# input-output-hk/plutus-halo2-verifier-gen

Hardware: AMD Instinct MI355X
Metric: halo2_proofs_verified_per_sec (higher is better)
Workload: dtype u32

## Files before the change

plutus_halo2_verifier_gen_amd/csrc/h2v_capi.hip:

```cpp
#include "../../include/h2v.h"

#include <hip/hip_runtime.h>
#include <stdio.h>
#include <stdlib.h>
#include <string.h>

#include <mutex>
#include <string>
#include <vector>

#include "h2v_kernels.hip"
#include "h2v_plancc.hpp"

static thread_local std::string g_err;
static int fail(int code, const std::string &msg) {
    g_err = msg;
    if (code == H2V_E_DEVICE && msg.find("hip: ") == std::string::npos) {
        const hipError_t e = hipPeekAtLastError();
        if (e != hipSuccess) g_err += std::string(" [hip: ") + hipGetErrorString(e) + "]";
    }
    return code;
}
#define HIPCHK(expr)                                                                                     \
    do {                                                                                                 \
// ... 53 lines not shown
        return fail(H2V_E_ARG, std::string("verifying-key description: ") + e.what());
    } catch (const std::exception &e) {
        return fail(H2V_E_ARG, std::string("plan compiler: ") + e.what());
    }
}
extern "C" void h2v_blob_free(uint8_t *blob) { free(blob); }

struct h2v_plan {
    int device = 0;
    bool dead = false;
    H2vDevPlan d{};
    void *blob = nullptr;
    void *fold_terms = nullptr;
    void *vk_tab = nullptr;
    void *fix_tab = nullptr;
    uint32_t n_var = 0, n_fix = 0;
    uint32_t n_squeezes = 0, stream_len = 0;
    uint64_t gen = 0;
    std::vector<uint32_t> trace_slots;
};

struct h2v_workspace {
    int device = 0;
    bool dead = false;
    uint32_t in_flight_hint = 1;
    bool hint_given = false;
    uint64_t cap = 0;
    uint32_t stride = 0;
    uint32_t sz_terms = 0, sz_slots = 0, sz_regs = 0 , sz_trace = 0;
    bool sz_ivc = false, sz_fix = false;
    uint32_t *regs = nullptr, *scalars = nullptr, *pts = nullptr, *er = nullptr, *status = nullptr, *trace = nullptr, *msm_tab = nullptr;
    uint32_t *accl = nullptr, *accr = nullptr, *fold_pts = nullptr, *fold_scal = nullptr, *el2 = nullptr, *er2 = nullptr;
    uint32_t *pt_tab = nullptr;
    uint32_t *er_fix = nullptr;
    uint32_t *msm_parts = nullptr;
// ... 264 lines not shown
        if (p->vk_tab) (void)hipFree(p->vk_tab);
        if (p->fold_terms) (void)hipFree(p->fold_terms);
        (void)hipFree(p->blob); delete p;
        return fail(H2V_E_DEVICE, "hipMalloc(vk tables) failed");
    }
    if (n_bases) {
        hipLaunchKernelGGL(k_vk_tables, dim3((n_bases + 63) / 64), dim3(64), 0, nullptr, d.vk_bases, n_bases, (uint32_t *)p->vk_tab);
        if (hipDeviceSynchronize() != hipSuccess) {
            (void)hipFree(p->vk_tab);
            if (p->fold_terms) (void)hipFree(p->fold_terms);
            (void)hipFree(p->blob); delete p;
            return fail(H2V_E_DEVICE, "VK window-table kernel failed");
        }
    }
    d.vk_tab = (const uint32_t *)p->vk_tab;
    if (!ivc && n_bases) {
        uint32_t nv = 0;
        while (nv < n_terms && rd32(patched.data() + w[H2V_HW_OFF_TERMS] + 8 * nv) != H2V_TERM_VK_BASE) nv++;
        bool tail_ok = nv < n_terms;
        for (uint32_t k = nv; k < n_terms; k++) tail_ok = tail_ok && rd32(patched.data() + w[H2V_HW_OFF_TERMS] + 8 * k) == H2V_TERM_VK_BASE;
        if (tail_ok) {
            uint32_t fc = (size_t)n_bases * 22 * 2048 * 112 <= ((size_t)2 << 30) ? 12u : 8u;
            if (opt_fix_c) fc = opt_fix_c;
            const uint32_t fW = fc == 4 ? 65u : fc == 8 ? 33u : 22u, fE = 1u << (fc - 1);
            const size_t fix_bytes = (size_t)n_bases * fW * fE * 28 * 4;
            void *wbase = nullptr;
            bool okf = hipMalloc(&p->fix_tab, fix_bytes + 16) == hipSuccess && hipMemset(p->fix_tab, 0, fix_bytes + 16) == hipSuccess &&
                       hipMalloc(&wbase, (size_t)n_bases * fW * 96 + 16) == hipSuccess;
            if (okf) {
                hipLaunchKernelGGL(k_vk_fixed_window_bases, dim3((n_bases * fW + 63) / 64), dim3(64), 0, nullptr, d.vk_bases, n_bases, fc, fW, (uint32_t *)wbase);
                const uint64_t entries = (uint64_t)n_bases * fW * fE;
                hipLaunchKernelGGL(k_vk_fixed_tables, dim3((uint32_t)((entries + 63) / 64)), dim3(64), 0, nullptr, (const uint32_t *)wbase, n_bases * fW, fc, (uint32_t *)p->fix_tab);
                okf = hipDeviceSynchronize() == hipSuccess;
            }
            if (wbase) (void)hipFree(wbase);
            d.fix_c = fc; d.fix_W = fW;
            if (!okf) {
                if (p->fix_tab) (void)hipFree(p->fix_tab);
                (void)hipFree(p->vk_tab);
                (void)hipFree(p->blob); delete p;
                return fail(H2V_E_DEVICE, "fixed-base table setup failed");
            }
            p->n_var = nv;
            p->n_fix = n_terms - nv;
        }
    }
    d.fix_tab = (const uint32_t *)p->fix_tab; d.n_var = p->n_var; d.n_fix = p->n_fix;
    p->n_squeezes = n_sq;
    p->stream_len = w[H2V_HW_STREAM_LEN];
    for (uint32_t k = 0; k < n_trace; k++) p->trace_slots.push_back(rd32(trp + 8 * k));
    { static std::mutex mu; static uint64_t loads = 0; std::lock_guard<std::mutex> lock(mu); p->gen = ++loads; }
    reg_add(g_plan_live, p);
    *out = p;
    return H2V_OK;
}
static void plan_release(h2v_plan *p) {
    (void)hipSetDevice(p->device);
    if (p->blob) (void)hipFree(p->blob);
    if (p->fold_terms) (void)hipFree(p->fold_terms);
    if (p->vk_tab) (void)hipFree(p->vk_tab);
    if (p->fix_tab) (void)hipFree(p->fix_tab);
    p->blob = p->fold_terms = p->vk_tab = p->fix_tab = nullptr;
}
extern "C" void h2v_plan_free(h2v_plan *p) {
    if (!p) return;
    reg_del(g_plan_live, p);
    if (!p->dead) plan_release(p);
    delete p;
}
extern "C" int h2v_plan_info(const h2v_plan *p, uint32_t *proof_len, uint32_t *n_pi, uint32_t *n_ci, uint32_t *n_terms) {
    if (!p) return fail(H2V_E_ARG, "null plan");
    if (proof_len) *proof_len = p->d.proof_len;
    if (n_pi) *n_pi = p->d.n_pi;
    if (n_ci) *n_ci = p->d.n_ci;
    if (n_terms) *n_terms = p->d.n_terms;
    return H2V_OK;
}
// ... 614 lines not shown
    return launch_msm_range(d, ma, n, scalars, pts, nullptr, st, in_flight_hint, seg);
}
struct IvcBufs { uint32_t *accl, *accr, *fold_pts, *fold_scal, *el2, *er2; };
static void launch_ivc_fold(const H2vDevPlan &d, uint32_t n, const uint32_t *pts, const uint32_t *er,
                            const IvcBufs &b, uint32_t *tabws, hipStream_t st) {
    hipLaunchKernelGGL(k_ivc_challenge, dim3((n + 63) / 64), dim3(64), 0, st, d, n, pts, er, b.accl, b.accr, b.fold_pts, b.fold_scal);
    const H2vMsmArgs fold = {d.fold_terms, 0, 4, 4, 0, 4, {2, 4, 4}, {b.el2, b.er2, nullptr}, nullptr, nullptr, nullptr, 0, 0};
    launch_msm_range(d, fold, n, b.fold_scal, b.fold_pts, tabws, st);
}
static uint32_t launch_pairing_impl(int impl, const H2vDevPlan &d, uint32_t n, const uint32_t *pts, const uint8_t *valid, const uint8_t *valid_sub, const uint32_t *er,
                                const uint32_t *el_jac, uint32_t *status, uint8_t *accept, uint32_t *dbg, hipStream_t st, const uint32_t *skip = nullptr,
                                bool prefer_narrow = false, double wide_up_to = -1.0, bool prefer_six = false, bool prefer_twelve = false) {
    if (wide_up_to < 0) wide_up_to = msm_n_simd();
    const int forced = g_opts.v[H2V_OPT_PAIRING_ENGINE];
    if (impl == 1 && forced) impl = forced == 1 ? 0 : forced == 16 ? 2 : forced == 64 ? 3 : forced == 6 ? 5 : forced == 12 ? 6 : 4;
    if (impl == 5 || (impl == 1 && !skip && prefer_six)) {
        hipLaunchKernelGGL(k_pairing_six, dim3((n + SIX_GROUPS - 1) / SIX_GROUPS), dim3(64), SIX_LDS_BYTES, st, d, n, pts, valid, valid_sub, er, el_jac, status, accept, dbg);
        return 6u;
    }
    const bool wide = !skip && impl != 2 && impl != 4 && impl != 6 && (impl == 3 || (double)n <= wide_up_to);
    const bool narrow = !skip && !wide && impl != 4 && (impl == 2 || prefer_narrow);
    if (impl == 6 || (narrow && impl != 2 && prefer_twelve)) {
        hipLaunchKernelGGL(k_pairing_coop_twelve, dim3((n + COOP_GROUPS_TWELVE - 1) / COOP_GROUPS_TWELVE), dim3(64), COOP_LDS_BYTES(COOP_GROUPS_TWELVE), st, d, n, pts, valid, valid_sub, er, el_jac, status, accept, dbg);
        return 12u;
    }
    if (impl == 0) { hipLaunchKernelGGL(k_pairing_check, dim3((n + 63) / 64), dim3(64), 0, st, d, n, pts, valid, valid_sub, er, el_jac, status, accept, dbg); return 1; }
    else if (wide) hipLaunchKernelGGL(k_pairing_coop_wide, dim3(n), dim3(64), COOP_LDS_BYTES(1), st, d, n, pts, valid, valid_sub, er, el_jac, status, accept, dbg);
    else if (narrow) hipLaunchKernelGGL(k_pairing_coop_narrow, dim3((n + 3) / 4), dim3(64), COOP_LDS_BYTES(COOP_GROUPS_NARROW), st, d, n, pts, valid, valid_sub, er, el_jac, status, accept, dbg);
    else hipLaunchKernelGGL(k_pairing_coop, dim3((n + 1) / 2), dim3(64), COOP_LDS_BYTES(COOP_GROUPS_PER_WAVE), st, d, n, pts, valid, valid_sub, er, el_jac, status, accept, dbg, skip);
    return wide ? 64u : narrow ? 16u : 32u;
}
// ... 1600 lines not shown
}
extern "C" int h2v_probe_pairing_ex(const h2v_plan *p, uint32_t n, const uint8_t *p1c, const uint8_t *p2c, uint8_t *out, int impl, uint8_t *dbg);
extern "C" int h2v_probe_pairing(const h2v_plan *p, uint32_t n, const uint8_t *p1c, const uint8_t *p2c, uint8_t *out) {
    return h2v_probe_pairing_ex(p, n, p1c, p2c, out, -1, nullptr);
}
extern "C" int h2v_probe_pairing_ex(const h2v_plan *p, uint32_t n, const uint8_t *p1c, const uint8_t *p2c, uint8_t *out, int impl, uint8_t *dbg) {
    if (!p || !p1c || !p2c || !out || n == 0) return fail(H2V_E_ARG, "bad argument");
    ALIVE(p);
    ProbeOpts probe_opts;
    DevBuf ddbg;
    HIPCHK(hipSetDevice(p->device));
    MiniPlan mp;
    DevBuf din, doff, dsc, dpts, dvalid, der, dst, dacc, dtab;
    mp.d.lines28_sg2 = p->d.lines28_sg2;
    mp.d.lines28_g2 = p->d.lines28_g2;
    if (mp.build(2, 1, p->d.lines_sg2, p->d.lines_g2) || upload_offsets(doff, n, 96) || din.alloc((size_t)n * 96) || dsc.alloc((size_t)n * 32) ||
        dpts.alloc((size_t)n * 192) || dvalid.alloc((size_t)n * 2) || der.alloc((size_t)n * 144) || dst.alloc((size_t)n * 4) || dacc.alloc(n))
        return fail(H2V_E_DEVICE, "probe setup failed");
    uint32_t term[2] = {H2V_TERM_PROOF_POINT, 1};
    HIPCHK(hipMemcpy(mp.terms.p, term, 8, hipMemcpyHostToDevice));
    std::vector<uint8_t> in((size_t)n * 96), one((size_t)n * 32, 0);
    for (uint32_t i = 0; i < n; i++) { memcpy(&in[(size_t)i * 96], p1c + (size_t)i * 48, 48); memcpy(&in[(size_t)i * 96 + 48], p2c + (size_t)i * 48, 48); one[(size_t)i * 32] = 1; }
    HIPCHK(hipMemcpy(din.p, in.data(), in.size(), hipMemcpyHostToDevice));
    HIPCHK(hipMemcpy(dsc.p, one.data(), one.size(), hipMemcpyHostToDevice));
    HIPCHK(hipMemset(dst.p, 0, (size_t)n * 4));
    if (dtab.alloc((size_t)n * 2 * 448 * 4)) return fail(H2V_E_DEVICE, "hipMalloc failed");
    hipLaunchKernelGGL(k_g1_decompress, dim3((n * 2 + 63) / 64), dim3(128), 0, nullptr, mp.d, n, din.as<uint8_t>(), doff.as<uint64_t>(), (const uint8_t *)nullptr, (const uint8_t *)nullptr, dpts.as<uint32_t>(), dvalid.as<uint8_t>(), dtab.as<uint32_t>(), 0u, (uint8_t *)nullptr);
    launch_msm(mp.d, n, dsc.as<uint32_t>(), dpts.as<uint32_t>(), dtab.as<uint32_t>(), der.as<uint32_t>(), nullptr, nullptr, nullptr);
    if (ddbg.alloc(dbg ? (size_t)n * 24 * 48 : 8)) return fail(H2V_E_DEVICE, "hipMalloc failed");
    launch_pairing_impl(impl, mp.d, n, dpts.as<uint32_t>(), dvalid.as<uint8_t>(), nullptr, der.as<uint32_t>(), nullptr, dst.as<uint32_t>(), dacc.as<uint8_t>(), dbg ? ddbg.as<uint32_t>() : nullptr, nullptr);
// ... 7 lines not shown
```

plutus_halo2_verifier_gen_amd/csrc/h2v_curve28.hpp:

```cpp
#pragma once
#include "h2v_curve.hpp"
#include "h2v_fp28.hpp"

struct G1J28 { F28 x, y, z; };

H2V_DI void g1j28_from_affine(G1J28 &r, const G1A &a) {
    f28_from_fp(r.x, a.x);
    f28_from_fp(r.y, a.y);
    f28_set_one(r.z);
}
H2V_DI void g1j28_to_g1j(G1J &r, const G1J28 &p, const bool inf) {
    if (inf) { g1j_set_inf(r); return; }
    F28 z = p.z;
    f28_carry(z);
    f28_to_fp(r.x, p.x);
    f28_to_fp(r.y, p.y);
    f28_to_fp(r.z, z);
}
#define F28_MUL_(r, a, b) do { if (INL) f28_mul_inl(r, a, b); else f28_mul(r, a, b); } while (0)
#define F28_SQR_(r, a) do { if (INL) f28_sqr_inl(r, a); else f28_sqr(r, a); } while (0)
template <bool INL>
H2V_DI void g1j28_dbl_t(G1J28 &r, const G1J28 &p) {
    F28 X = p.x, Y = p.y, Z = p.z, A, B, D, t;
    F28_NEG(t, Y, 21, 1);
// ... 3 lines not shown
    F28_MUL_(D, X, B);
    f28_mul_small<3>(A, A);
    F28_SQR_(X, A);
    f28_mul_small<8>(t, D);
    F28_SUB(X, X, t, 17, 8); f28_carry(X);
    f28_mul_small<4>(D, D);
    F28_SUB(t, X, D, 9, 4); f28_carry(t);
    f28_mul_small<2>(B, B);
    if (INL) f28_dot2_sqr_inl<2>(Y, B, A, t);
    else f28_dot2_sqr<2>(Y, B, A, t);
    r.x = X; r.y = Y; r.z = Z;
}
#undef F28_MUL_
#undef F28_SQR_
H2V_DI void g1j28_dbl(G1J28 &r, const G1J28 &p) { g1j28_dbl_t<false>(r, p); }
H2V_DI int g1j28_add(G1J28 &r, const G1J28 &p, const G1J28 &q, const bool neg_q) {
    F28 X1 = p.x, Y1 = p.y, Z1 = p.z, a, b, c, t;
    f28_sqr(a, q.z);
    f28_mul(X1, X1, a);
    f28_mul(t, q.z, a); f28_mul(Y1, Y1, t);
    f28_sqr(a, Z1);
    f28_mul(b, q.x, a);
    f28_mul(t, Z1, a);
    {
        F28 qy = q.y, nq;
        F28_NEG(nq, qy, 20, 1);
        if (neg_q) qy = nq;
        f28_mul(c, qy, t);
    }
    F28_SUB(b, b, X1, 3, 1); f28_carry(b);
    F28_SUB(c, Y1, c, 3, 1); f28_carry(c);
    if (f28_is_zero_v5(b)) {
        if (f28_is_zero_v5(c)) { g1j28_dbl(r, p); return 1; }
        return 2;
    }
    f28_mul(Z1, Z1, q.z); f28_mul(Z1, Z1, b);
    f28_sqr(a, b);
    F28_NEG(t, a, 3, 1);
    f28_mul(b, b, t);
    f28_mul(a, X1, t);
    f28_sqr(X1, c);
    f28_add(X1, X1, b);
    f28_mul_small<2>(t, a);
    f28_add(X1, X1, t); f28_carry(X1);
    f28_add(t, a, X1);
    f28_dot2(Y1, c, t, Y1, b);
    r.x = X1; r.y = Y1; r.z = Z1;
    return 0;
}
#define F28_MUL_(r, a, b) do { if (INL) f28_mul_inl(r, a, b); else f28_mul(r, a, b); } while (0)
#define F28_SQR_(r, a) do { if (INL) f28_sqr_inl(r, a); else f28_sqr(r, a); } while (0)
// ... 212 lines not shown
        f28_mul(bx, x, b28);
        g1_store_table_entry(tab2 + 224 + m * 28, bx, y);
    }
}
H2V_DI void g1j28_acc_add(G1J28 &acc, bool &acc_inf, const G1J28 &q, const bool neg) {
    if (acc_inf) {
        acc = q;
        if (neg) { F28 ny; F28_NEG(ny, q.y, 20, 1); f28_carry(ny); acc.y = ny; }
        acc_inf = false;
        return;
    }
    const int k = g1j28_add(acc, acc, q, neg);
    if (k == 2) acc_inf = true;
}

H2V_DN void g1j28_mul_x_abs(G1J28 &r, bool &r_inf, const G1J28 &p, const bool p_inf) {
    G1J28 acc = p;
    bool inf = p_inf;
#pragma unroll 1
    for (int i = 62; i >= 0; i--) {
        if (!inf) g1j28_dbl_t<true>(acc, acc);
        if (((BLS_X_ABS >> i) & 1) && !p_inf) g1j28_acc_add(acc, inf, p, false);
    }
    r = acc;
    r_inf = inf;
}
H2V_DN bool g1a_in_subgroup28(const G1A &a) {
    G1J28 p, t;
    bool tinf = false;
    g1j28_from_affine(p, a);
    g1j28_mul_x_abs(t, tinf, p, false);
    g1j28_mul_x_abs(t, tinf, t, tinf);
    if (tinf) return false;
    G1J tj;
    g1j28_to_g1j(tj, t, false);
    Fp beta, z2, z3, l, ny;
#pragma unroll
    for (int i = 0; i < 12; i++) beta.v[i] = FP_BETA[i];
    fp_sqr(z2, tj.z);
    fp_mul(z3, z2, tj.z);
    fp_mul(l, a.x, beta); fp_mul(l, l, z2);
    if (!fp_eq(l, tj.x)) return false;
    fp_mul(l, a.y, z3);
    fp_neg(ny, tj.y);
    return fp_eq(l, ny);
}
```

plutus_halo2_verifier_gen_amd/csrc/h2v_pairing_six.hpp:

```cpp
#pragma once
#include "h2v_pairing_coop.hpp"
#include "six_tables.h"

#define H2V_NO_TAIL_MARK __attribute__((disable_tail_calls))
#define SIX_GROUPS 10
#define SIX_SLOT_DW 14
#define SIX_GROUP_DW (SIX_N_GROUP_SLOTS * SIX_SLOT_DW)
#define SIX_TAB_DW ((6 * 4 * SIX_N_MUL + 6 * 4 * SIX_N_SQR + 2 * 6 * 4 * SIX_N_LINE + 6 * 16) / 4)
#define SIX_TAB_OFF (SIX_N_SHARED_SLOTS * SIX_SLOT_DW)
#define SIX_GRP_OFF ((SIX_TAB_OFF + SIX_TAB_DW + 1) & ~1)
#define SIX_LDS_BYTES ((size_t)(SIX_GRP_OFF + SIX_GROUPS * SIX_GROUP_DW) * 4)
#define SIX_TAB_MUL_B 0
#define SIX_TAB_SQR_B (6 * 4 * SIX_N_MUL)
#define SIX_TAB_LINE1_B (SIX_TAB_SQR_B + 6 * 4 * SIX_N_SQR)
#define SIX_TAB_LINE2_B (SIX_TAB_LINE1_B + 6 * 4 * SIX_N_LINE)
#define SIX_TAB_CSQR_B (SIX_TAB_LINE2_B + 6 * 4 * SIX_N_LINE)
#define SIX_C_M(k) ((k) < 3 ? 19 + (k) : 31 + (k))

struct Six {
    int grp_off;
    int k;
    bool act;
};
struct SixF2 { F28 re, im; };
// ... 63 lines not shown
            r.l[k] = (uint32_t)carry & FP28_MASK;
            carry >>= 28;
        }
        r.l[13] = (uint32_t)(carry + (int64_t)acc[27] + (int64_t)FP_MOD28[13]);
    } else {
        uint64_t carry = 0;
#pragma unroll
        for (int k = 0; k < 13; k++) {
            carry += acc[14 + k];
            r.l[k] = (uint32_t)carry & FP28_MASK;
            carry >>= 28;
        }
        r.l[13] = (uint32_t)(carry + acc[27]);
    }
}
H2V_DN void six_kara(const Six c, const int tab_row_byte, const int nt, const bool keep) {
    const uint8_t *tab = reinterpret_cast<const uint8_t *>(coop_lds + SIX_TAB_OFF) + tab_row_byte;
    uint64_t U[28], V[28], W[28];
#pragma unroll
    for (int i = 0; i < 28; i++) { U[i] = 0; V[i] = 0; W[i] = 0; }
#pragma unroll 1
    for (int t = 0; t < nt; t++) {
        uint32_t x0[14], y0[14], x1[14], y1[14];
        six_load_pair(x0, y0, six_slot(c, tab[4 * t]), six_slot(c, tab[4 * t + 1]));
        six_mac(U, x0, y0);
        six_load_pair(x1, y1, six_slot(c, tab[4 * t + 2]), six_slot(c, tab[4 * t + 3]));
        six_mac(V, x1, y1);
#pragma unroll
        for (int i = 0; i < 14; i++) { x1[i] += x0[i]; y1[i] += y0[i]; }
        six_mac(W, x1, y1);
    }
#pragma unroll
    for (int i = 0; i < 27; i++) {
        W[i] -= U[i] + V[i];
        U[i] -= V[i];
    }
    SixF2 r;
    six_reduce<false>(r.im, W);
    six_reduce<true>(r.re, U);
    if (c.act && !keep) {
        six_store(six_slot(c, SIX_SLOT_A + 2 * c.k), r.re);
        six_store(six_slot(c, SIX_SLOT_A + 2 * c.k + 1), r.im);
    }
}
H2V_DN void six_csqr_engine(const Six c, const int tab_row_byte) {
    const uint8_t *tab = reinterpret_cast<const uint8_t *>(coop_lds + SIX_TAB_OFF) + tab_row_byte;
    uint64_t U[28], V[28], W[28];
#pragma unroll
    for (int i = 0; i < 28; i++) { U[i] = 0; V[i] = 0; W[i] = 0; }
    uint32_t x[14], x2[14], y[14];
// ... 34 lines not shown
    six_reduce<false>(r, acc);
    return f28_pack(r);
}
H2V_DI SixF2 six_result(const Six &c, const int base) {
    SixF2 r;
    six_load_pair(r.re.l, r.im.l, six_slot(c, base + 2 * c.k), six_slot(c, base + 2 * c.k + 1));
    return r;
}
H2V_DI SixF2 six_unpack(const SixRegs &z) {
    SixF2 r;
    r.re = f28_unpack(z.re.a, z.re.b, z.re.c, z.re.d);
    r.im = f28_unpack(z.im.a, z.im.b, z.im.c, z.im.d);
    return r;
}

H2V_DI void six_stage_a(const Six &c, const SixF2 &a, const int xa_from) {
    if (!c.act) return;
    six_store(six_slot(c, SIX_SLOT_A + 2 * c.k), a.re);
    six_store(six_slot(c, SIX_SLOT_A + 2 * c.k + 1), a.im);
    if (c.k >= xa_from) {
        F28 t, x0, x1;
        F28_NEG(t, a.im, 7, 1);
        f28_add(x0, a.re, t);
        f28_carry(x0);
        f28_add(x1, a.re, a.im);
        f28_carry(x1);
        six_store(six_slot(c, SIX_SLOT_XA + 2 * (c.k - 1)), x0);
        six_store(six_slot(c, SIX_SLOT_XA + 2 * (c.k - 1) + 1), x1);
    }
}
H2V_DI void six_stage_b(const Six &c, const SixF2 &b) {
    if (!c.act) return;
    six_store(six_slot(c, SIX_SLOT_B + 2 * c.k), b.re);
    six_store(six_slot(c, SIX_SLOT_B + 2 * c.k + 1), b.im);
}
H2V_DI void six_stage_d(const Six &c, const SixF2 &a) {
    if (!c.act) return;
    F28 d0, d1;
    f28_mul_small<2>(d0, a.re);
    f28_mul_small<2>(d1, a.im);
    six_store(six_slot(c, SIX_SLOT_B + 2 * c.k), d0);
    six_store(six_slot(c, SIX_SLOT_B + 2 * c.k + 1), d1);
}
H2V_DI SixF2 six_mul(const Six &c, const SixF2 &a, const SixF2 &b) {
    six_stage_a(c, a, 1);
    six_stage_b(c, b);
    __syncthreads();
    six_kara(c, SIX_TAB_MUL_B + c.k * 4 * SIX_N_MUL, SIX_N_MUL, false);
    __syncthreads();
    return six_result(c, SIX_SLOT_A);
}
H2V_DI SixF2 six_sqr(const Six &c, const SixF2 &a) {
    six_stage_a(c, a, 3);
    six_stage_d(c, a);
    __syncthreads();
    six_kara(c, SIX_TAB_SQR_B + c.k * 4 * SIX_N_SQR, SIX_N_SQR, false);
    __syncthreads();
    return six_result(c, SIX_SLOT_A);
}
template <int LOOP>
H2V_DI SixF2 six_line(const Six &c, const SixF2 &f, const bool skip) {
    six_stage_a(c, f, 3);
    __syncthreads();
    six_kara(c, (LOOP == 1 ? SIX_TAB_LINE1_B : SIX_TAB_LINE2_B) + c.k * 4 * SIX_N_LINE, SIX_N_LINE, skip);
    __syncthreads();
    return six_result(c, SIX_SLOT_A);
}
H2V_DI SixF2 six_csqr(const Six &c, const SixF2 &a) {
    if (c.act) {
        F28 na, d0, d1, m;
        F28_NEG(na, a.im, 7, 1);
        f28_add(m, a.re, na);
        f28_carry(na);
        f28_carry(m);
        f28_mul_small<2>(d0, a.re);
        f28_mul_small<2>(d1, a.im);
        six_store(six_slot(c, SIX_SLOT_A + 2 * c.k), a.re);
        six_store(six_slot(c, SIX_SLOT_A + 2 * c.k + 1), a.im);
        six_store(six_slot(c, SIX_SLOT_C_NA + c.k), na);
// ... 6 lines not shown
            six_store(six_slot(c, SIX_SLOT_C_ND2), nd);
        }
    }
    __syncthreads();
    six_csqr_engine(c, SIX_TAB_CSQR_B + c.k * 16);
    __syncthreads();
    SixF2 r = six_result(c, SIX_SLOT_B);
    const SixF2 g = six_result(c, SIX_SLOT_A);
    const bool minus = (c.k & 1) == 0;
#pragma unroll
    for (int i = 0; i < 14; i++) {
        const uint32_t g0 = g.re.l[i] << 1, g1 = g.im.l[i] << 1;
        r.re.l[i] = 3u * r.re.l[i] + (minus ? F28_BIAS_13_2[i] - g0 : g0);
        r.im.l[i] = 3u * r.im.l[i] + (minus ? F28_BIAS_13_2[i] - g1 : g1);
    }
    f28_carry(r.re);
    f28_carry(r.im);
    f28_fold(r.re);
    f28_fold(r.im);
    return r;
}
H2V_DI SixF2 six_conj(const Six &c, const SixF2 &a) {
    SixF2 r = a;
    if (c.k & 1) {
        F28_NEG(r.re, a.re, 6, 1);
        F28_NEG(r.im, a.im, 6, 1);
        f28_carry(r.re);
        f28_carry(r.im);
    }
    return r;
}
H2V_DI SixF2 six_frob(const Six &c, const SixF2 &a) {
// ... 23 lines not shown
    f28_to_fp(z.c1, nn.im);
    fp_set_zero(zi.c0);
    fp_set_zero(zi.c1);
    bool good = true;
    if (c.k == 0) good = fp2_inv(zi, z);
    ok = good;
    SixF2 ninv;
    f28_from_fp(ninv.re, zi.c0);
    f28_from_fp(ninv.im, zi.c1);
    const SixF2 r = six_mul(c, fc, six_mul(c, adj, ninv));
    SixRegs o;
    o.re = f28_pack(r.re);
    o.im = f28_pack(r.im);
    return o;
}
H2V_DI uint2 six_line_share(const uint32_t *lines28, int idx, int lane) {
    return reinterpret_cast<const uint2 *>(lines28 + (size_t)idx * 8 * 16)[lane];
}
H2V_DI void six_line_store(int shared_slot, const uint2 v, int lane) {
    if ((lane & 7) == 7) return;
    uint32_t *dst = coop_lds + (shared_slot - SIX_SHARED_BASE + (lane >> 3)) * SIX_SLOT_DW + 2 * (lane & 7);
    dst[0] = v.x;
    dst[1] = v.y;
}

extern "C" __global__ void __launch_bounds__(64, 2) H2V_NO_TAIL_MARK
k_pairing_six(H2vDevPlan plan, uint32_t n, const uint32_t *__restrict__ pts, const uint8_t *__restrict__ valid, const uint8_t *__restrict__ valid_sub,
              const uint32_t *__restrict__ er_jac, const uint32_t *__restrict__ el_jac ,
              uint32_t *__restrict__ status, uint8_t *__restrict__ accept, uint32_t *__restrict__ dbg) {
    const int lane = threadIdx.x;
    const int grp6 = (lane * 43) >> 8;
    Six c;
    c.act = lane < 6 * SIX_GROUPS;
    const int grp = c.act ? grp6 : SIX_GROUPS - 1;
    c.k = c.act ? lane - 6 * grp6 : lane - 6 * SIX_GROUPS;
    c.grp_off = SIX_GRP_OFF + grp * SIX_GROUP_DW;
// ... 57 lines not shown
        if (op == COOP_OP_END) break;
        switch (op) {
        case COOP_OP_MUL: {
            const SixF2 x = vars[a], y = vars[b];
            vars[d] = six_mul(c, x, y);
        } break;
        case COOP_OP_CSQR: {
            SixF2 x = vars[a];
#pragma unroll 1
            for (int rep = 0; rep < b; rep++) x = six_csqr(c, x);
            vars[d] = x;
        } break;
        case COOP_OP_MILLER: {
            SixF2 f = vars[COOP_VAR_F];
            int ln = 0;
            uint2 c1 = six_line_share(plan.lines28_sg2, 0, lane), c2 = six_line_share(plan.lines28_g2, 0, lane);
#pragma unroll 1
            for (int bit = 62; bit >= 0; bit--) {
                f = six_sqr(c, f);
                const int steps = ((BLS_X_ABS >> bit) & 1) ? 2 : 1;
#pragma unroll 1
                for (int s2 = 0; s2 < steps; s2++, ln++) {
                    six_line_store(SIX_SLOT_LN1, c1, lane);
                    six_line_store(SIX_SLOT_LN2, c2, lane);
                    if (ln + 1 < H2V_MILLER_LINES) { c1 = six_line_share(plan.lines28_sg2, ln + 1, lane); c2 = six_line_share(plan.lines28_g2, ln + 1, lane); }
                    __syncthreads();
                    {
                        const int u = (c.k >> 1) & 1, part = c.k & 1;
                        const F28Regs z = six_prod(c, (u ? SIX_SLOT_LN2 : SIX_SLOT_LN1) + part, u ? SIX_SLOT_PX2 : SIX_SLOT_PX1);
                        if (c.act && c.k < 4) six_store(six_slot(c, (u ? SIX_SLOT_T2 : SIX_SLOT_T1) + part), f28_unpack(z.a, z.b, z.c, z.d));
                    }
                    f = six_line<1>(c, f, skip1);
                    f = six_line<2>(c, f, skip2);
                }
            }
            vars[COOP_VAR_F] = f;
        } break;
        case COOP_OP_EXPX: {
            SixF2 x = vars[a];
#pragma unroll 1
            for (int bit = 62; bit >= 0; bit--) {
                x = six_csqr(c, x);
                if ((BLS_X_ABS >> bit) & 1) {
                    const SixF2 y = vars[a];
                    x = six_mul(c, x, y);
                }
            }
            vars[d] = six_conj(c, x);
        } break;
        case COOP_OP_WARMUP: break;
// ... 5 lines not shown
            fr.re = f28_pack(vars[a].re);
            fr.im = f28_pack(vars[a].im);
            vars[d] = six_unpack(six_inv_raw(c, fr, ok));
            inv_ok = ok;
        } break;
        case COOP_OP_MOV: vars[d] = vars[a]; break;
        case COOP_OP_SETONE: {
            SixF2 o;
            f28_set_zero(o.re);
            f28_set_zero(o.im);
            if (c.k == 0) f28_set_one(o.re);
            vars[d] = o;
        } break;
        case COOP_OP_DUMP: {
            if (dbg && live && c.act) {
                Fp o, oc;
                f28_to_fp(oc, vars[a].re);
                fp_from_mont(o, oc);
#pragma unroll
                for (int q = 0; q < 12; q++) dbg[((size_t)i * 24 + 12 * d + 2 * c.k) * 12 + q] = o.v[q];
                f28_to_fp(oc, vars[a].im);
                fp_from_mont(o, oc);
#pragma unroll
                for (int q = 0; q < 12; q++) dbg[((size_t)i * 24 + 12 * d + 2 * c.k + 1) * 12 + q] = o.v[q];
            }
        } break;
        default: break;
        }
    }
    Fp res0, res1;
    f28_to_fp(res0, vars[COOP_VAR_F].re);
    f28_to_fp(res1, vars[COOP_VAR_F].im);
    bool mine = fp_is_zero(res1);
    if (c.k == 0) { Fp one; fp_set_one(one); mine = mine && fp_eq(res0, one); }
    else mine = mine && fp_is_zero(res0);
    const unsigned long long bal = __ballot(mine);
    const bool is_one = ((bal >> leader) & 0x3full) == 0x3full;
// ... 8 lines not shown
```

plutus_halo2_verifier_gen_amd/csrc/h2v_plan.h:

```cpp
#pragma once
#include <stdint.h>

#define H2V_PLAN_MAGIC "H2VPLAN1"
#define H2V_PLAN_VERSION 4u
#define H2V_PLAN_HDR_WORDS 46
#define H2V_MILLER_LINES 68

enum {
    H2V_HW_VERSION = 0, H2V_HW_PROOF_LEN, H2V_HW_N_PI, H2V_HW_N_CI, H2V_HW_N_REGS, H2V_HW_N_INSTR, H2V_HW_N_CONSTS,
    H2V_HW_N_POINTS, H2V_HW_N_VK_BASES, H2V_HW_N_TERMS, H2V_HW_N_TRACE, H2V_HW_PI_POINT, H2V_HW_N_SQUEEZES,
    H2V_HW_STREAM_LEN,
    H2V_HW_OFF_INSTR, H2V_HW_OFF_CONSTS, H2V_HW_OFF_POINTS, H2V_HW_OFF_VK_BASES, H2V_HW_OFF_TERMS, H2V_HW_OFF_LINES_SG2,
    H2V_HW_OFF_LINES_G2, H2V_HW_OFF_TRACE, H2V_HW_TOTAL_LEN, H2V_HW_OFF_LINES28_SG2, H2V_HW_OFF_LINES28_G2,
    H2V_HW_IVC, H2V_HW_N_MAIN_TERMS, H2V_HW_ACC_IDX0 ,
    H2V_HW_VM_LANES = H2V_HW_ACC_IDX0 + 8, H2V_HW_VM2_LANES, H2V_HW_VM2_N_REGS, H2V_HW_VM2_N_INSTR, H2V_HW_VM2_OFF_INSTR
};

enum {
    H2V_OP_END = 0, H2V_OP_ABSORB_REG, H2V_OP_ABSORB_CI, H2V_OP_LOAD_INSTANCE, H2V_OP_READ_POINT, H2V_OP_READ_SCALAR,
    H2V_OP_SQUEEZE, H2V_OP_CONST, H2V_OP_ADD, H2V_OP_SUB, H2V_OP_MUL, H2V_OP_NEG, H2V_OP_INV, H2V_OP_OUT_SCALAR,
    H2V_OP_ASSERT_ZERO,
    H2V_OP_NOP,
    H2V_OP_COUNT
};
// ... 15 lines not shown
    uint16_t dst, a, b;
};

struct H2vDevPlan {
    uint32_t proof_len, n_pi, n_ci, n_regs, n_instr, n_consts, n_points, n_vk_bases, n_terms, n_trace, pi_point;
    uint32_t vm_lanes;
    const H2vInstr *instr;
    const uint32_t *consts;
    const uint32_t *points;
    const uint32_t *vk_bases;
    const uint32_t *terms;
    const uint32_t *lines_sg2;
    const uint32_t *lines_g2;
    const uint32_t *lines28_sg2;
    const uint32_t *lines28_g2;
    const uint32_t *trace;
    uint32_t ivc, n_main_terms;
    uint32_t acc_idx[8];
    const uint32_t *fold_terms;
    const uint32_t *vk_tab;
    const uint32_t *fix_tab;
    uint32_t n_var, n_fix;
    uint32_t fix_c, fix_W;
    uint32_t wide_lanes, wide_n_regs, wide_n_instr;
    const H2vInstr *wide_instr;
};
#define H2V_SLOTS(plan) ((plan).n_points + (plan).n_ci + 2u * (plan).ivc)
```

plutus_halo2_verifier_gen_amd/csrc/six_tables.h:

```cpp
#pragma once
#include <stdint.h>
#define SIX_SLOT_A 0
#define SIX_SLOT_XA 12
#define SIX_SLOT_T1 22
#define SIX_SLOT_T2 24
#define SIX_SLOT_B 22
#define SIX_SLOT_C_NA 12
#define SIX_SLOT_C_ND2 18
#define SIX_SLOT_PX1 34
#define SIX_SLOT_PY1 35
#define SIX_SLOT_PX2 36
#define SIX_SLOT_PY2 37
#define SIX_SLOT_ZERO 82
#define SIX_SLOT_LN1 64
#define SIX_SLOT_LN2 72
#define SIX_SLOT_C23P 80
#define SIX_SLOT_C23N 81
#define SIX_N_GROUP_SLOTS 38
#define SIX_N_SHARED_SLOTS 19
#define SIX_SHARED_BASE 64
#define SIX_N_MUL 6
#define SIX_N_SQR 4
#define SIX_N_LINE 3
#define SIX_N_CSQR 5
__device__ alignas(4) static constexpr uint8_t SIX_TAB_MUL[6][24] = {
    {0, 22, 1, 23, 12, 32, 13, 33, 14, 30, 15, 31, 16, 28, 17, 29, 18, 26, 19, 27, 20, 24, 21, 25},
    {0, 24, 1, 25, 2, 22, 3, 23, 14, 32, 15, 33, 16, 30, 17, 31, 18, 28, 19, 29, 20, 26, 21, 27},
    {0, 26, 1, 27, 2, 24, 3, 25, 4, 22, 5, 23, 16, 32, 17, 33, 18, 30, 19, 31, 20, 28, 21, 29},
    {0, 28, 1, 29, 2, 26, 3, 27, 4, 24, 5, 25, 6, 22, 7, 23, 18, 32, 19, 33, 20, 30, 21, 31},
    {0, 30, 1, 31, 2, 28, 3, 29, 4, 26, 5, 27, 6, 24, 7, 25, 8, 22, 9, 23, 20, 32, 21, 33},
    {0, 32, 1, 33, 2, 30, 3, 31, 4, 28, 5, 29, 6, 26, 7, 27, 8, 24, 9, 25, 10, 22, 11, 23}};
__device__ alignas(4) static constexpr uint8_t SIX_TAB_SQR[6][16] = {
    {0, 0, 1, 1, 24, 20, 25, 21, 26, 18, 27, 19, 6, 16, 7, 17},
    {0, 24, 1, 25, 26, 20, 27, 21, 28, 18, 29, 19, 82, 82, 82, 82},
    {0, 26, 1, 27, 2, 2, 3, 3, 28, 20, 29, 21, 8, 18, 9, 19},
    {0, 28, 1, 29, 2, 26, 3, 27, 30, 20, 31, 21, 82, 82, 82, 82},
    {0, 30, 1, 31, 2, 28, 3, 29, 4, 4, 5, 5, 10, 20, 11, 21},
    {0, 32, 1, 33, 2, 30, 3, 31, 4, 28, 5, 29, 82, 82, 82, 82}};
__device__ alignas(4) static constexpr uint8_t SIX_TAB_LINE1[6][12] = {
    {0, 68, 1, 69, 18, 22, 19, 23, 16, 35, 17, 82},
    {2, 68, 3, 69, 20, 22, 21, 23, 18, 35, 19, 82},
    {4, 68, 5, 69, 0, 22, 1, 23, 20, 35, 21, 82},
    {6, 68, 7, 69, 2, 22, 3, 23, 0, 35, 1, 82},
    {8, 68, 9, 69, 4, 22, 5, 23, 2, 35, 3, 82},
    {10, 68, 11, 69, 6, 22, 7, 23, 4, 35, 5, 82}};
__device__ alignas(4) static constexpr uint8_t SIX_TAB_LINE2[6][12] = {
    {0, 76, 1, 77, 18, 24, 19, 25, 16, 37, 17, 82},
    {2, 76, 3, 77, 20, 24, 21, 25, 18, 37, 19, 82},
    {4, 76, 5, 77, 0, 24, 1, 25, 20, 37, 21, 82},
    {6, 76, 7, 77, 2, 24, 3, 25, 0, 37, 1, 82},
    {8, 76, 9, 77, 4, 24, 5, 25, 2, 37, 3, 82},
    {10, 76, 11, 77, 6, 24, 7, 25, 4, 37, 5, 82}};
__device__ alignas(4) static constexpr uint8_t SIX_TAB_CSQR[6][16] = {
    {0, 1, 19, 6, 7, 34, 6, 82, 29, 0, 82, 23, 6, 7, 34, 82},
    {26, 82, 36, 10, 11, 18, 82, 82, 82, 10, 11, 26, 27, 82, 36, 82},
    {2, 3, 20, 8, 9, 35, 8, 82, 31, 2, 82, 25, 8, 9, 35, 82},
    {0, 82, 28, 12, 82, 29, 82, 82, 82, 0, 82, 29, 1, 82, 28, 82},
    {4, 5, 21, 10, 11, 36, 10, 82, 33, 4, 82, 27, 10, 11, 36, 82},
    {2, 82, 30, 13, 82, 31, 82, 82, 82, 2, 82, 31, 3, 82, 30, 82}};
```

Baseline: 1.296 million.

## Normalize Miller line coefficients on host to cut six-lane line products

At plan load, the host precomputes normalized Miller-loop line coefficients by dividing each line by its constant term. It also records the accumulated scale factors, which are only reapplied in the debug dump path. The six-lane pairing kernel's line multiplication then uses two Karatsuba products instead of three, adding the Fp12 value directly, and loads one shared line record per step instead of two. Separately, the G1 x-multiplication subgroup check now uses a mixed affine add for the first pass and a cached z^2/z^3 add for the second, and a redundant carry is dropped. The risks are a changed final-exponentiation input, since the scale factors are in a subfield that the final exponentiation kills, and new bias bounds in the staging step.

```diff
diff --git a/plutus_halo2_verifier_gen_amd/csrc/h2v_capi.hip b/plutus_halo2_verifier_gen_amd/csrc/h2v_capi.hip
--- a/plutus_halo2_verifier_gen_amd/csrc/h2v_capi.hip
+++ b/plutus_halo2_verifier_gen_amd/csrc/h2v_capi.hip
@@ -91,11 +91,70 @@
     void *fold_terms = nullptr;
     void *vk_tab = nullptr;
     void *fix_tab = nullptr;
+    void *six_tab = nullptr;
     uint32_t n_var = 0, n_fix = 0;
     uint32_t n_squeezes = 0, stream_len = 0;
     uint64_t gen = 0;
     std::vector<uint32_t> trace_slots;
 };
+
+#define SIX_NORM_DW (H2V_MILLER_LINES * 2 * 4 * 16)
+static bool six_line_tables(const uint8_t *l28_sg2, const uint8_t *l28_g2, std::vector<uint32_t> &out) {
+    using namespace h2vhost;
+    U384 c376;
+    c376.w[5] = (uint64_t)1 << (376 - 320);
+    auto slot_fp = [&](const uint8_t *slot) {
+        U384 m;
+        for (int i = 0; i < 14; i++) {
+            uint32_t limb;
+            memcpy(&limb, slot + 4 * i, 4);
+            const int bit = 28 * i;
+            m.w[bit >> 6] |= (uint64_t)limb << (bit & 63);
+            if ((bit & 63) > 36 && (bit >> 6) + 1 < 6) m.w[(bit >> 6) + 1] |= (uint64_t)limb >> (64 - (bit & 63));
+        }
+        return FpE{FP().mul(m, c376)};
+    };
+    auto put_slot = [&](uint32_t *dst, const FpE &a) {
+        uint8_t b[48];
+        fp_mont392_bytes(a, b);
+        U384 m;
+        memcpy(m.w, b, 48);
+        for (int i = 0; i < 14; i++) {
+            const int bit = 28 * i;
+            uint64_t v = m.w[bit >> 6] >> (bit & 63);
+            if ((bit & 63) > 36 && (bit >> 6) + 1 < 6) v |= m.w[(bit >> 6) + 1] << (64 - (bit & 63));
+            dst[i] = (uint32_t)(v & 0xfffffffu);
+        }
+        dst[14] = dst[15] = 0;
+    };
+    auto put_words = [&](uint32_t *dst, const FpE &a) {
+        uint8_t b[48];
+        fp_mont392_bytes(a, b);
+        memcpy(dst, b, 48);
+    };
+    out.assign(SIX_NORM_DW + 4 * 24, 0);
+    const uint8_t *src[2] = {l28_sg2, l28_g2};
+    F2 K[2] = {f2_one(), f2_one()};
+    int ln = 0;
+    for (int bit = 62; bit >= 0; bit--) {
+        const int steps = ((0xd201000000010000ull >> bit) & 1) ? 2 : 1;
+        for (int u = 0; u < 2; u++) K[u] = f2_sqr(K[u]);
+        for (int s2 = 0; s2 < steps; s2++, ln++)
+            for (int u = 0; u < 2; u++) {
+                const uint8_t *rec = src[u] + (size_t)ln * 8 * 64;
+                const F2 nl = {slot_fp(rec), slot_fp(rec + 64)}, cc = {slot_fp(rec + 4 * 64), slot_fp(rec + 5 * 64)};
+                if (f2_is_zero(cc)) return false;
+                const F2 B = f2_inv(cc), A = f2_mul(nl, B);
+                uint32_t *dst = out.data() + ((size_t)ln * 2 + u) * 4 * 16;
+                put_slot(dst, A.a); put_slot(dst + 16, A.b); put_slot(dst + 32, B.a); put_slot(dst + 48, B.b);
+                K[u] = f2_mul(K[u], cc);
+            }
+    }
+    if (ln != H2V_MILLER_LINES) return false;
+    const F2 ks[4] = {f2_one(), K[0], K[1], f2_mul(K[0], K[1])};
+    for (int q = 0; q < 4; q++) { put_words(out.data() + SIX_NORM_DW + 24 * q, ks[q].a); put_words(out.data() + SIX_NORM_DW + 24 * q + 12, ks[q].b); }
+    return true;
+}
 
 struct h2v_workspace {
     int device = 0;
@@ -390,6 +449,20 @@
         }
     }
     d.vk_tab = (const uint32_t *)p->vk_tab;
+    {
+        std::vector<uint32_t> six;
+        if (six_line_tables(blob + w[H2V_HW_OFF_LINES28_SG2], blob + w[H2V_HW_OFF_LINES28_G2], six)) {
+            if (hipMalloc(&p->six_tab, six.size() * 4) != hipSuccess || hipMemcpy(p->six_tab, six.data(), six.size() * 4, hipMemcpyHostToDevice) != hipSuccess) {
+                if (p->six_tab) (void)hipFree(p->six_tab);
+                (void)hipFree(p->vk_tab);
+                if (p->fold_terms) (void)hipFree(p->fold_terms);
+                (void)hipFree(p->blob); delete p;
+                return fail(H2V_E_DEVICE, "six-lane line table upload failed");
+            }
+            d.six_norm28 = (const uint32_t *)p->six_tab;
+            d.six_k = d.six_norm28 + SIX_NORM_DW;
+        }
+    }
     if (!ivc && n_bases) {
         uint32_t nv = 0;
         while (nv < n_terms && rd32(patched.data() + w[H2V_HW_OFF_TERMS] + 8 * nv) != H2V_TERM_VK_BASE) nv++;
@@ -413,6 +486,7 @@
             d.fix_c = fc; d.fix_W = fW;
             if (!okf) {
                 if (p->fix_tab) (void)hipFree(p->fix_tab);
+                if (p->six_tab) (void)hipFree(p->six_tab);
                 (void)hipFree(p->vk_tab);
                 (void)hipFree(p->blob); delete p;
                 return fail(H2V_E_DEVICE, "fixed-base table setup failed");
@@ -436,7 +510,8 @@
     if (p->fold_terms) (void)hipFree(p->fold_terms);
     if (p->vk_tab) (void)hipFree(p->vk_tab);
     if (p->fix_tab) (void)hipFree(p->fix_tab);
-    p->blob = p->fold_terms = p->vk_tab = p->fix_tab = nullptr;
+    if (p->six_tab) (void)hipFree(p->six_tab);
+    p->blob = p->fold_terms = p->vk_tab = p->fix_tab = p->six_tab = nullptr;
 }
 extern "C" void h2v_plan_free(h2v_plan *p) {
     if (!p) return;
@@ -1081,7 +1156,7 @@
     if (wide_up_to < 0) wide_up_to = msm_n_simd();
     const int forced = g_opts.v[H2V_OPT_PAIRING_ENGINE];
     if (impl == 1 && forced) impl = forced == 1 ? 0 : forced == 16 ? 2 : forced == 64 ? 3 : forced == 6 ? 5 : forced == 12 ? 6 : 4;
-    if (impl == 5 || (impl == 1 && !skip && prefer_six)) {
+    if ((impl == 5 || (impl == 1 && !skip && prefer_six)) && d.six_norm28) {
         hipLaunchKernelGGL(k_pairing_six, dim3((n + SIX_GROUPS - 1) / SIX_GROUPS), dim3(64), SIX_LDS_BYTES, st, d, n, pts, valid, valid_sub, er, el_jac, status, accept, dbg);
         return 6u;
     }
@@ -2712,6 +2787,8 @@
     DevBuf din, doff, dsc, dpts, dvalid, der, dst, dacc, dtab;
     mp.d.lines28_sg2 = p->d.lines28_sg2;
     mp.d.lines28_g2 = p->d.lines28_g2;
+    mp.d.six_norm28 = p->d.six_norm28;
+    mp.d.six_k = p->d.six_k;
     if (mp.build(2, 1, p->d.lines_sg2, p->d.lines_g2) || upload_offsets(doff, n, 96) || din.alloc((size_t)n * 96) || dsc.alloc((size_t)n * 32) ||
         dpts.alloc((size_t)n * 192) || dvalid.alloc((size_t)n * 2) || der.alloc((size_t)n * 144) || dst.alloc((size_t)n * 4) || dacc.alloc(n))
         return fail(H2V_E_DEVICE, "probe setup failed");
diff --git a/plutus_halo2_verifier_gen_amd/csrc/h2v_curve28.hpp b/plutus_halo2_verifier_gen_amd/csrc/h2v_curve28.hpp
--- a/plutus_halo2_verifier_gen_amd/csrc/h2v_curve28.hpp
+++ b/plutus_halo2_verifier_gen_amd/csrc/h2v_curve28.hpp
@@ -41,11 +41,10 @@
 #undef F28_MUL_
 #undef F28_SQR_
 H2V_DI void g1j28_dbl(G1J28 &r, const G1J28 &p) { g1j28_dbl_t<false>(r, p); }
-H2V_DI int g1j28_add(G1J28 &r, const G1J28 &p, const G1J28 &q, const bool neg_q) {
+H2V_DI int g1j28_add_zz(G1J28 &r, const G1J28 &p, const G1J28 &q, const bool neg_q, const F28 &zz, const F28 &zzz) {
     F28 X1 = p.x, Y1 = p.y, Z1 = p.z, a, b, c, t;
-    f28_sqr(a, q.z);
-    f28_mul(X1, X1, a);
-    f28_mul(t, q.z, a); f28_mul(Y1, Y1, t);
+    f28_mul(X1, X1, zz);
+    f28_mul(Y1, Y1, zzz);
     f28_sqr(a, Z1);
     f28_mul(b, q.x, a);
     f28_mul(t, Z1, a);
@@ -62,6 +61,39 @@
         return 2;
     }
     f28_mul(Z1, Z1, q.z); f28_mul(Z1, Z1, b);
+    f28_sqr(a, b);
+    F28_NEG(t, a, 3, 1);
+    f28_mul(b, b, t);
+    f28_mul(a, X1, t);
+    f28_sqr(X1, c);
+    f28_add(X1, X1, b);
+    f28_mul_small<2>(t, a);
+    f28_add(X1, X1, t); f28_carry(X1);
+    f28_add(t, a, X1);
+    f28_dot2(Y1, c, t, Y1, b);
+    r.x = X1; r.y = Y1; r.z = Z1;
+    return 0;
+}
+H2V_DI int g1j28_add(G1J28 &r, const G1J28 &p, const G1J28 &q, const bool neg_q) {
+    F28 zz, zzz;
+    f28_sqr(zz, q.z);
+    f28_mul(zzz, q.z, zz);
+    return g1j28_add_zz(r, p, q, neg_q, zz, zzz);
+}
+H2V_DI int g1j28_madd_complete(G1J28 &r, const G1J28 &p, const F28 &qx, const F28 &qy) {
+    F28 X1 = p.x, Y1 = p.y, Z1 = p.z, a, b, c, t;
+    f28_sqr(a, Z1);
+    f28_mul(b, qx, a);
+    f28_mul(t, Z1, a);
+    f28_mul(c, qy, t);
+    F28_SUB(b, b, X1, 20, 1);
+    f28_fold(b);
+    F28_SUB(c, Y1, c, 3, 1); f28_carry(c);
+    if (f28_is_zero_v5(b)) {
+        if (f28_is_zero_v5(c)) { g1j28_dbl(r, p); return 1; }
+        return 2;
+    }
+    f28_mul(Z1, Z1, b);
     f28_sqr(a, b);
     F28_NEG(t, a, 3, 1);
     f28_mul(b, b, t);
@@ -304,13 +336,29 @@
     if (k == 2) acc_inf = true;
 }
 
+template <bool AFFINE>
 H2V_DN void g1j28_mul_x_abs(G1J28 &r, bool &r_inf, const G1J28 &p, const bool p_inf) {
     G1J28 acc = p;
     bool inf = p_inf;
+    F28 zz, zzz;
+    f28_set_zero(zz);
+    f28_set_zero(zzz);
+    if (!AFFINE && !p_inf) {
+        f28_sqr(zz, p.z);
+        f28_mul(zzz, p.z, zz);
+    }
 #pragma unroll 1
     for (int i = 62; i >= 0; i--) {
         if (!inf) g1j28_dbl_t<true>(acc, acc);
-        if (((BLS_X_ABS >> i) & 1) && !p_inf) g1j28_acc_add(acc, inf, p, false);
+        if (((BLS_X_ABS >> i) & 1) && !p_inf) {
+            if (inf) {
+                acc = p;
+                inf = false;
+            } else {
+                const int k = AFFINE ? g1j28_madd_complete(acc, acc, p.x, p.y) : g1j28_add_zz(acc, acc, p, false, zz, zzz);
+                if (k == 2) inf = true;
+            }
+        }
     }
     r = acc;
     r_inf = inf;
@@ -319,8 +367,8 @@
     G1J28 p, t;
     bool tinf = false;
     g1j28_from_affine(p, a);
-    g1j28_mul_x_abs(t, tinf, p, false);
-    g1j28_mul_x_abs(t, tinf, t, tinf);
+    g1j28_mul_x_abs<true>(t, tinf, p, false);
+    g1j28_mul_x_abs<false>(t, tinf, t, tinf);
     if (tinf) return false;
     G1J tj;
     g1j28_to_g1j(tj, t, false);
diff --git a/plutus_halo2_verifier_gen_amd/csrc/h2v_pairing_six.hpp b/plutus_halo2_verifier_gen_amd/csrc/h2v_pairing_six.hpp
--- a/plutus_halo2_verifier_gen_amd/csrc/h2v_pairing_six.hpp
+++ b/plutus_halo2_verifier_gen_amd/csrc/h2v_pairing_six.hpp
@@ -101,7 +101,7 @@
         r.l[13] = (uint32_t)(carry + acc[27]);
     }
 }
-H2V_DN void six_kara(const Six c, const int tab_row_byte, const int nt, const bool keep) {
+H2V_DN void six_kara(const Six c, const int tab_row_byte, const int nt, const bool keep, const bool addself) {
     const uint8_t *tab = reinterpret_cast<const uint8_t *>(coop_lds + SIX_TAB_OFF) + tab_row_byte;
     uint64_t U[28], V[28], W[28];
 #pragma unroll
@@ -121,6 +121,12 @@
     for (int i = 0; i < 27; i++) {
         W[i] -= U[i] + V[i];
         U[i] -= V[i];
+    }
+    if (addself) {
+        uint32_t f0[14], f1[14];
+        six_load_pair(f0, f1, six_slot(c, SIX_SLOT_A + 2 * c.k), six_slot(c, SIX_SLOT_A + 2 * c.k + 1));
+#pragma unroll
+        for (int i = 0; i < 14; i++) { U[14 + i] += f0[i]; W[14 + i] += f1[i]; }
     }
     SixF2 r;
     six_reduce<false>(r.im, W);
@@ -185,13 +191,16 @@
     return r;
 }
 
+template <bool MILLER = false>
 H2V_DI void six_stage_a(const Six &c, const SixF2 &a, const int xa_from) {
     if (!c.act) return;
     six_store(six_slot(c, SIX_SLOT_A + 2 * c.k), a.re);
     six_store(six_slot(c, SIX_SLOT_A + 2 * c.k + 1), a.im);
     if (c.k >= xa_from) {
         F28 t, x0, x1;
-        F28_NEG(t, a.im, 7, 1);
+        static_assert(SIX_MILLER_K == 11, "the bias table of the Miller loop's staging");
+        if (MILLER) F28_NEG(t, a.im, 11, 1);
+        else F28_NEG(t, a.im, 7, 1);
         f28_add(x0, a.re, t);
         f28_carry(x0);
         f28_add(x1, a.re, a.im);
@@ -217,23 +226,23 @@
     six_stage_a(c, a, 1);
     six_stage_b(c, b);
     __syncthreads();
-    six_kara(c, SIX_TAB_MUL_B + c.k * 4 * SIX_N_MUL, SIX_N_MUL, false);
+    six_kara(c, SIX_TAB_MUL_B + c.k * 4 * SIX_N_MUL, SIX_N_MUL, false, false);
     __syncthreads();
     return six_result(c, SIX_SLOT_A);
 }
 H2V_DI SixF2 six_sqr(const Six &c, const SixF2 &a) {
-    six_stage_a(c, a, 3);
+    six_stage_a<true>(c, a, 3);
     six_stage_d(c, a);
     __syncthreads();
-    six_kara(c, SIX_TAB_SQR_B + c.k * 4 * SIX_N_SQR, SIX_N_SQR, false);
+    six_kara(c, SIX_TAB_SQR_B + c.k * 4 * SIX_N_SQR, SIX_N_SQR, false, false);
     __syncthreads();
     return six_result(c, SIX_SLOT_A);
 }
 template <int LOOP>
 H2V_DI SixF2 six_line(const Six &c, const SixF2 &f, const bool skip) {
-    six_stage_a(c, f, 3);
-    __syncthreads();
-    six_kara(c, (LOOP == 1 ? SIX_TAB_LINE1_B : SIX_TAB_LINE2_B) + c.k * 4 * SIX_N_LINE, SIX_N_LINE, skip);
+    six_stage_a<true>(c, f, 3);
+    __syncthreads();
+    six_kara(c, (LOOP == 1 ? SIX_TAB_LINE1_B : SIX_TAB_LINE2_B) + c.k * 4 * SIX_N_LINE, SIX_N_LINE, skip, true);
     __syncthreads();
     return six_result(c, SIX_SLOT_A);
 }
@@ -270,8 +279,6 @@
         r.re.l[i] = 3u * r.re.l[i] + (minus ? F28_BIAS_13_2[i] - g0 : g0);
         r.im.l[i] = 3u * r.im.l[i] + (minus ? F28_BIAS_13_2[i] - g1 : g1);
     }
-    f28_carry(r.re);
-    f28_carry(r.im);
     f28_fold(r.re);
     f28_fold(r.im);
     return r;
@@ -325,12 +332,13 @@
     o.im = f28_pack(r.im);
     return o;
 }
-H2V_DI uint2 six_line_share(const uint32_t *lines28, int idx, int lane) {
-    return reinterpret_cast<const uint2 *>(lines28 + (size_t)idx * 8 * 16)[lane];
-}
-H2V_DI void six_line_store(int shared_slot, const uint2 v, int lane) {
+H2V_DI uint2 six_line_share(const uint32_t *norm28, int idx, int lane) {
+    return reinterpret_cast<const uint2 *>(norm28 + (size_t)idx * 8 * 16)[lane];
+}
+H2V_DI void six_line_store(const uint2 v, int lane) {
+    static_assert(SIX_SLOT_LN2 == SIX_SLOT_LN1 + 4, "the two loops' constants are one run of eight slots");
     if ((lane & 7) == 7) return;
-    uint32_t *dst = coop_lds + (shared_slot - SIX_SHARED_BASE + (lane >> 3)) * SIX_SLOT_DW + 2 * (lane & 7);
+    uint32_t *dst = coop_lds + (SIX_SLOT_LN1 - SIX_SHARED_BASE + (lane >> 3)) * SIX_SLOT_DW + 2 * (lane & 7);
     dst[0] = v.x;
     dst[1] = v.y;
 }
@@ -418,26 +426,31 @@
         case COOP_OP_MILLER: {
             SixF2 f = vars[COOP_VAR_F];
             int ln = 0;
-            uint2 c1 = six_line_share(plan.lines28_sg2, 0, lane), c2 = six_line_share(plan.lines28_g2, 0, lane);
+            uint2 cn = six_line_share(plan.six_norm28, 0, lane);
+            const int u = (c.k >> 1) & 1, part = c.k & 1;
+            const int xs1 = c.k < 4 ? (u ? SIX_SLOT_LN2 : SIX_SLOT_LN1) + part : SIX_SLOT_LN1 + 2 + part;
+            const int ys1 = c.k < 4 ? (u ? SIX_SLOT_PX2 : SIX_SLOT_PX1) : SIX_SLOT_PY1;
 #pragma unroll 1
             for (int bit = 62; bit >= 0; bit--) {
                 f = six_sqr(c, f);
                 const int steps = ((BLS_X_ABS >> bit) & 1) ? 2 : 1;
 #pragma unroll 1
                 for (int s2 = 0; s2 < steps; s2++, ln++) {
-                    six_line_store(SIX_SLOT_LN1, c1, lane);
-                    six_line_store(SIX_SLOT_LN2, c2, lane);
-                    if (ln + 1 < H2V_MILLER_LINES) { c1 = six_line_share(plan.lines28_sg2, ln + 1, lane); c2 = six_line_share(plan.lines28_g2, ln + 1, lane); }
+                    six_line_store(cn, lane);
+                    if (ln + 1 < H2V_MILLER_LINES) cn = six_line_share(plan.six_norm28, ln + 1, lane);
                     __syncthreads();
                     {
-                        const int u = (c.k >> 1) & 1, part = c.k & 1;
-                        const F28Regs z = six_prod(c, (u ? SIX_SLOT_LN2 : SIX_SLOT_LN1) + part, u ? SIX_SLOT_PX2 : SIX_SLOT_PX1);
-                        if (c.act && c.k < 4) six_store(six_slot(c, (u ? SIX_SLOT_T2 : SIX_SLOT_T1) + part), f28_unpack(z.a, z.b, z.c, z.d));
+                        F28Regs z = six_prod(c, xs1, ys1);
+                        if (c.act) six_store(six_slot(c, SIX_SLOT_T + c.k), f28_unpack(z.a, z.b, z.c, z.d));
+                        z = six_prod(c, SIX_SLOT_LN2 + 2 + part, SIX_SLOT_PY2);
+                        if (c.act && c.k < 2) six_store(six_slot(c, SIX_SLOT_T + 6 + c.k), f28_unpack(z.a, z.b, z.c, z.d));
                     }
                     f = six_line<1>(c, f, skip1);
                     f = six_line<2>(c, f, skip2);
                 }
             }
+            f28_fold(f.re);
+            f28_fold(f.im);
             vars[COOP_VAR_F] = f;
         } break;
         case COOP_OP_EXPX: {
@@ -473,13 +486,22 @@
         } break;
         case COOP_OP_DUMP: {
             if (dbg && live && c.act) {
-                Fp o, oc;
-                f28_to_fp(oc, vars[a].re);
-                fp_from_mont(o, oc);
+                Fp2 v;
+                f28_to_fp(v.c0, vars[a].re);
+                f28_to_fp(v.c1, vars[a].im);
+                if (d == 0) {
+                    const uint32_t *kp = plan.six_k + ((skip1 ? 0 : 1) + (skip2 ? 0 : 2)) * 24;
+                    Fp2 kk, t;
+#pragma unroll
+                    for (int q = 0; q < 12; q++) { kk.c0.v[q] = kp[q]; kk.c1.v[q] = kp[12 + q]; }
+                    fp2_mul(t, v, kk);
+                    v = t;
+                }
+                Fp o;
+                fp_from_mont(o, v.c0);
 #pragma unroll
                 for (int q = 0; q < 12; q++) dbg[((size_t)i * 24 + 12 * d + 2 * c.k) * 12 + q] = o.v[q];
-                f28_to_fp(oc, vars[a].im);
-                fp_from_mont(o, oc);
+                fp_from_mont(o, v.c1);
 #pragma unroll
                 for (int q = 0; q < 12; q++) dbg[((size_t)i * 24 + 12 * d + 2 * c.k + 1) * 12 + q] = o.v[q];
             }
diff --git a/plutus_halo2_verifier_gen_amd/csrc/h2v_plan.h b/plutus_halo2_verifier_gen_amd/csrc/h2v_plan.h
--- a/plutus_halo2_verifier_gen_amd/csrc/h2v_plan.h
+++ b/plutus_halo2_verifier_gen_amd/csrc/h2v_plan.h
@@ -53,6 +53,8 @@
     const uint32_t *lines_g2;
     const uint32_t *lines28_sg2;
     const uint32_t *lines28_g2;
+    const uint32_t *six_norm28;
+    const uint32_t *six_k;
     const uint32_t *trace;
     uint32_t ivc, n_main_terms;
     uint32_t acc_idx[8];
diff --git a/plutus_halo2_verifier_gen_amd/csrc/six_tables.h b/plutus_halo2_verifier_gen_amd/csrc/six_tables.h
--- a/plutus_halo2_verifier_gen_amd/csrc/six_tables.h
+++ b/plutus_halo2_verifier_gen_amd/csrc/six_tables.h
@@ -2,8 +2,7 @@
 #include <stdint.h>
 #define SIX_SLOT_A 0
 #define SIX_SLOT_XA 12
-#define SIX_SLOT_T1 22
-#define SIX_SLOT_T2 24
+#define SIX_SLOT_T 22
 #define SIX_SLOT_B 22
 #define SIX_SLOT_C_NA 12
 #define SIX_SLOT_C_ND2 18
@@ -13,7 +12,7 @@
 #define SIX_SLOT_PY2 37
 #define SIX_SLOT_ZERO 82
 #define SIX_SLOT_LN1 64
-#define SIX_SLOT_LN2 72
+#define SIX_SLOT_LN2 68
 #define SIX_SLOT_C23P 80
 #define SIX_SLOT_C23N 81
 #define SIX_N_GROUP_SLOTS 38
@@ -21,8 +20,9 @@
 #define SIX_SHARED_BASE 64
 #define SIX_N_MUL 6
 #define SIX_N_SQR 4
-#define SIX_N_LINE 3
+#define SIX_N_LINE 2
 #define SIX_N_CSQR 5
+#define SIX_MILLER_K 11
 __device__ alignas(4) static constexpr uint8_t SIX_TAB_MUL[6][24] = {
     {0, 22, 1, 23, 12, 32, 13, 33, 14, 30, 15, 31, 16, 28, 17, 29, 18, 26, 19, 27, 20, 24, 21, 25},
     {0, 24, 1, 25, 2, 22, 3, 23, 14, 32, 15, 33, 16, 30, 17, 31, 18, 28, 19, 29, 20, 26, 21, 27},
@@ -37,20 +37,20 @@
     {0, 28, 1, 29, 2, 26, 3, 27, 30, 20, 31, 21, 82, 82, 82, 82},
     {0, 30, 1, 31, 2, 28, 3, 29, 4, 4, 5, 5, 10, 20, 11, 21},
     {0, 32, 1, 33, 2, 30, 3, 31, 4, 28, 5, 29, 82, 82, 82, 82}};
-__device__ alignas(4) static constexpr uint8_t SIX_TAB_LINE1[6][12] = {
-    {0, 68, 1, 69, 18, 22, 19, 23, 16, 35, 17, 82},
-    {2, 68, 3, 69, 20, 22, 21, 23, 18, 35, 19, 82},
-    {4, 68, 5, 69, 0, 22, 1, 23, 20, 35, 21, 82},
-    {6, 68, 7, 69, 2, 22, 3, 23, 0, 35, 1, 82},
-    {8, 68, 9, 69, 4, 22, 5, 23, 2, 35, 3, 82},
-    {10, 68, 11, 69, 6, 22, 7, 23, 4, 35, 5, 82}};
-__device__ alignas(4) static constexpr uint8_t SIX_TAB_LINE2[6][12] = {
-    {0, 76, 1, 77, 18, 24, 19, 25, 16, 37, 17, 82},
-    {2, 76, 3, 77, 20, 24, 21, 25, 18, 37, 19, 82},
-    {4, 76, 5, 77, 0, 24, 1, 25, 20, 37, 21, 82},
-    {6, 76, 7, 77, 2, 24, 3, 25, 0, 37, 1, 82},
-    {8, 76, 9, 77, 4, 24, 5, 25, 2, 37, 3, 82},
-    {10, 76, 11, 77, 6, 24, 7, 25, 4, 37, 5, 82}};
+__device__ alignas(4) static constexpr uint8_t SIX_TAB_LINE1[6][8] = {
+    {18, 22, 19, 23, 16, 26, 17, 27},
+    {20, 22, 21, 23, 18, 26, 19, 27},
+    {0, 22, 1, 23, 20, 26, 21, 27},
+    {2, 22, 3, 23, 0, 26, 1, 27},
+    {4, 22, 5, 23, 2, 26, 3, 27},
+    {6, 22, 7, 23, 4, 26, 5, 27}};
+__device__ alignas(4) static constexpr uint8_t SIX_TAB_LINE2[6][8] = {
+    {18, 24, 19, 25, 16, 28, 17, 29},
+    {20, 24, 21, 25, 18, 28, 19, 29},
+    {0, 24, 1, 25, 20, 28, 21, 29},
+    {2, 24, 3, 25, 0, 28, 1, 29},
+    {4, 24, 5, 25, 2, 28, 3, 29},
+    {6, 24, 7, 25, 4, 28, 5, 29}};
 __device__ alignas(4) static constexpr uint8_t SIX_TAB_CSQR[6][16] = {
     {0, 1, 19, 6, 7, 34, 6, 82, 29, 0, 82, 23, 6, 7, 34, 82},
     {26, 82, 36, 10, 11, 18, 82, 82, 82, 10, 11, 26, 27, 82, 36, 82},
```

Measured after the change: 1.327 million, median of 6. 2.4% higher.
